# bernardomig/torch_semantic_segmentation

Measured on AMD Instinct MI355X. Metric: images/sec (train step) fastscnn 1024x2048 bs=8, higher is better.
Workload: dtype bf16; 1 GPU; fastscnn train step (zero_grad+fwd+CE(ignore 255)+bwd+AdamW), 8 x 3 x 1024 x 2048 per GPU, 19 classes, random-init weights; global_batch=8, parallelism=dp1, hip_graph=True, syncbn=False

## Files before the change

include/tss_hip.h:

```cpp
#ifndef TSS_HIP_H
#define TSS_HIP_H

#ifdef __cplusplus
extern "C" {
#endif

#define TSS_OK 0
#define TSS_ERR_DTYPE (-1)
#define TSS_ERR_SHAPE (-2)
#define TSS_ERR_ALIGN (-3)
#define TSS_ERR_HIP (-4)

#define TSS_F32 0
#define TSS_BF16 1

typedef struct tss_bn_bwd_job {
  const double* bstats; double count; const float* invstd; const float* gamma; int training; int accumulate;
  float* dgamma; float* dbeta; float* ga; float* gb; float* gce; int C;
  int xchg_world; int xchg_rank; void* xchg_peers[8]; void* xchg_counters;
} tss_bn_bwd_job;

enum {
  TSS_K_PWCONV_FWD = 0, TSS_K_PWCONV_BWD_DATA, TSS_K_PWCONV_BWD_WEIGHT,
  TSS_K_CONV3X3_FWD, TSS_K_CONV3X3_BWD_DATA, TSS_K_CONV3X3_BWD_WEIGHT,
  TSS_K_STEM_FWD, TSS_K_STEM_BWD_WEIGHT,
  TSS_K_DWCONV_FWD, TSS_K_DWCONV_BWD_DATA, TSS_K_DWCONV_BWD_WEIGHT,
  TSS_K_BN_FINALIZE, TSS_K_BN_BWD_FINALIZE, TSS_K_JOIN_FWD, TSS_K_JOIN_BWD,
  TSS_K_DROPOUT, TSS_K_BIAS_GRAD, TSS_K_ADAMW,
  TSS_K_BILINEAR_FWD, TSS_K_BILINEAR_BWD, TSS_K_BILINEAR_BWD_COLS, TSS_K_BILINEAR_PLANAR_FWD,
  TSS_K_UPSAMPLE_HEAD_FWD, TSS_K_UPSAMPLE_HEAD_BWD_ROWS, TSS_K_UPSAMPLE_HEAD_BWD_COLS,
  TSS_K_POOL_FWD, TSS_K_POOL_BWD, TSS_K_COPY,
  TSS_K_CE_FWD, TSS_K_CE_BWD, TSS_K_ARGMAX, TSS_K_UPSAMPLE_CE_FWD, TSS_K_UPSAMPLE_CE_BWD,
  TSS_K_RESIZE_FLIP_PLANAR, TSS_K_MULTISCALE_ARGMAX,
  TSS_K_SGD, TSS_K_GRAD_NORM,
  TSS_K_WIDE_CE_FWD, TSS_K_WIDE_CE_BWD, TSS_K_WIDE_ARGMAX, TSS_K_WIDE_MULTISCALE_ARGMAX,
  TSS_K_COUNT
};

int tss_version(void);
int tss_memset_zero(void* p, long bytes, void* stream);
const char* tss_last_error(void);
const char* tss_arch(void);
#define TSS_OPT_DISABLE_FAST_PATHS 1
int tss_set_option(int key, int value);
int tss_get_option(int key);

int tss_prof_enable(int on);
int tss_prof_reset(void);
int tss_prof_collect(void);
int tss_prof_get(int kernel_id, long* launches, double* total_ms, double* alg_bytes, double* flops);
long tss_prof_records(int* kernel_ids, double* ms, double* alg_bytes, long max_records);
const char* tss_prof_name(int kernel_id);
const char* tss_prof_symbol(int kernel_id);

int tss_pwconv_fwd(const void* x, long ldx, const float* in_mean, const float* in_scale, const float* in_bias, int in_relu,
                   const float* w, const void* w_bf16, const float* bias, void* y, long ldy, double* stats,
                   long P, int K, int N, int dtype, void* stream);
int tss_pwconv_fwd_joined(const void* x, long ldx, const float* in_mean, const float* in_scale, const float* in_bias, int in_relu,
// ... 210 lines not shown
int tss_bn_eval_affine(const float* gamma, const float* running_mean, const float* running_var,
                       float eps, float* mean_out, float* invstd_out, float* scale, int C, void* stream);
int tss_bn_eval_affine_batched(const long long* table, int njobs, int max_channels, void* stream);
int tss_bn_bwd_finalize(const double* bstats, double count, const float* invstd,
                        const float* gamma, int training, int accumulate, float* dgamma, float* dbeta,
                        float* ga, float* gb, float* gce, int C, void* stream);

int tss_slab_reduce(const double* slabs, double count, double* out, int C, void* stream);
int tss_bn_finalize_sync(const double* gsums, const float* gamma, float eps, float momentum, float* running_mean,
                         float* running_var, long long* num_batches_tracked, float* mean_out, float* invstd_out,
                         float* scale, int C, void* stream);
int tss_bn_bwd_finalize_sync(const double* bstats, const double* gsums, const float* invstd, const float* gamma,
                             int accumulate, float* dgamma, float* dbeta, float* ga, float* gb, float* gce, int C,
                             void* stream);

int tss_join_fwd(const void* a, long lda, const float* ma, const float* sa, const float* ba,
                 const void* b, long ldb, const float* mb, const float* sb, const float* bb,
                 void* out, long ldo, int relu, float drop_p, const unsigned long long* seed_slot,
                 long P, int C, int dtype, void* stream);
int tss_join_bwd(const void* dout, long lddo, const void* out, long ldo, int relu,
                 const void* a_raw, long lda, const float* mean_a, double* stats_a,
                 const void* b_raw, long ldb, const float* mean_b, double* stats_b,
                 void* e, long lde, float dout_scale, long P, int C, int dtype, void* stream);

int tss_dropout_tick(unsigned long long* counter, unsigned long long* seed_slot, void* stream);
int tss_dropout(const void* x, long ldx, void* y, long ldy, long P, int C, float p,
                const unsigned long long* seed_slot, int dtype, void* stream);
int tss_bias_grad(const void* e, long lde, long P, int N, float* dbias, int dtype, void* stream);
int tss_dropout_mask(const unsigned long long* counter, void* mask, long P, int C, float p, void* stream);
int tss_pwconv_drop_supported(long P, int K, int N, int dtype);
int tss_pwconv_fwd_drop(const void* x, long ldx, const float* in_mean, const float* in_scale, const float* in_bias, int in_relu,
                        const float* w, const void* w_bf16, const float* bias, void* y, long ldy,
                        const void* mask, float drop_p, unsigned long long* counter,
                        long P, int K, int N, int dtype, void* stream);
int tss_pwconv_bwd_fused_drop_supported(long P, int Cin, int Cout, int dtype);
int tss_pwconv_bwd_fused_drop_rows(long P);
int tss_pwconv_bwd_fused_drop(const void* e, long lde, const void* yraw, long ldyr, const float* ga, const float* gb, const float* gce,
                              const float* gmu, const float* w, const void* x, long ldx, const float* in_mean,
                              const float* in_scale, const float* in_bias, int in_relu, int x_pending, const void* mask, float drop_p,
                              void* e_in, long ldei, double* bstats, float* ws, float* bias_ws, long P, int Cin, int Cout, int dtype,
                              void* stream);
int tss_cast_weights(const long long* table, int njobs, int blocks_per_job, float* zero, long zero_n, void* stream);
int tss_adamw_step(float* params, const float* grads, float* exp_avg, float* exp_avg_sq, long n,
                   const float* lr, float beta1, float beta2, float eps, float weight_decay,
                   float* state, float grad_scale, float lr_host, long step_host, void* stream);

// ... 170 lines not shown
```

torch_semantic_segmentation_amd/_native.py:

```python
import ctypes
import os

import torch

_HERE = os.path.dirname(os.path.abspath(__file__))
LIB_PATH = os.environ.get('TSS_HIP_LIB') or os.path.join(_HERE, 'libtss_hip.so')

TSS_F32, TSS_BF16 = 0, 1
ERRORS = {-1: 'TSS_ERR_DTYPE (unsupported dtype)', -2: 'TSS_ERR_SHAPE (unsupported shape or pitch)',
          -3: 'TSS_ERR_ALIGN (pointer not 16-byte aligned)', -4: 'TSS_ERR_HIP (HIP launch error)'}

_P, _L, _I, _F, _D = ctypes.c_void_p, ctypes.c_long, ctypes.c_int, ctypes.c_float, ctypes.c_double

HEADER_PATH = os.path.join(os.path.dirname(_HERE), 'include', 'tss_hip.h')


def parse_header(path=HEADER_PATH):
    import re
    text = open(path).read()
    text = re.sub(r'/\*.*?\*/', ' ', text, flags=re.S)
    scalars = {'int': _I, 'long': _L, 'float': _F, 'double': _D}
    decls = {}
    for m in re.finditer(r'\b(int|long|const\s+char\s*\*)\s*(tss_\w+)\s*\(([^)]*)\)\s*;', text):
        ret, name, params = m.group(1), m.group(2), m.group(3).strip()
# ... 47 lines not shown
def stream():
    return torch.cuda.current_stream().cuda_stream


_slabs = None


def stat_slabs():
    global _slabs
    if _slabs is None:
        _slabs = lib().tss_stat_slabs()
    return _slabs


def dtype_code(dtype):
    if dtype == torch.float32:
        return TSS_F32
    if dtype == torch.bfloat16:
        return TSS_BF16
    raise TypeError('the HIP path computes in float32 or bfloat16 activations, got %s' % dtype)



K_COUNT = 41


def prof_enable(on=True):
    call('tss_prof_enable', 1 if on else 0)


def prof_reset():
    call('tss_prof_reset')


def prof_records(limit=100000):
    h = lib()
    ids = (ctypes.c_int * limit)()
    ms = (ctypes.c_double * limit)()
    by = (ctypes.c_double * limit)()
    n = min(h.tss_prof_records(ids, ms, by, limit), limit)
    return [(h.tss_prof_name(ids[i]).decode(), ms[i], by[i]) for i in range(n)]


def prof_table():
    call('tss_prof_collect')
    out = {}
    h = lib()
# ... 8 lines not shown
```

torch_semantic_segmentation_amd/csrc/bnfin.h:

```cpp
#pragma once
#include "common.h"

namespace tss_fin {

constexpr int FIN_CH = 8, FIN_RG = 4, FIN_WAVES = 4, FIN_NT = FIN_WAVES * 64;
static_assert(2 * FIN_CH * FIN_RG == 64, "one wave = row groups x 2 columns x channels");
__device__ __forceinline__ void slab_sum(const double* slabs, int C, int blk, double* s0, double* s1, int* c_out) {
  __shared__ double red[FIN_WAVES][64];
  const int lane = threadIdx.x & 63, wave = threadIdx.x >> 6;
  const int cl = lane & (FIN_CH - 1), hs = (lane / FIN_CH) & 1, rg = lane / (2 * FIN_CH);
  const int c = blk * FIN_CH + cl;
  const bool in = c < C;
  const double* col = slabs + (long)hs * C + (in ? c : 0);
  constexpr int RSTEP = FIN_WAVES * FIN_RG;
  constexpr int R = TSS_STAT_SLABS / RSTEP;
  static_assert(TSS_STAT_SLABS % RSTEP == 0, "slab rows must divide evenly");
  double acc = 0.0;
  double v[R];
#pragma unroll
  for (int u = 0; u < R; ++u) v[u] = col[(long)(wave * FIN_RG + rg + RSTEP * u) * 2 * C];
#pragma unroll
  for (int u = 0; u < R; ++u) acc += v[u];
  red[wave][lane] = in ? acc : 0.0;
  __syncthreads();
  double a = 0.0, b = 0.0;
  if (threadIdx.x < FIN_CH) {
#pragma unroll
    for (int w = 0; w < FIN_WAVES; ++w)
#pragma unroll
      for (int q = 0; q < FIN_RG; ++q) {
        a += red[w][q * 2 * FIN_CH + threadIdx.x];
        b += red[w][q * 2 * FIN_CH + FIN_CH + threadIdx.x];
      }
  }
  *s0 = a; *s1 = b; *c_out = blk * FIN_CH + threadIdx.x;
}


constexpr int XMAXB = 96;
constexpr int XCELL = 18;
constexpr int XSLOTS = 4;
constexpr int XMAXW = 8;
constexpr long XHEAD = 8;

__host__ __device__ inline long cell_off(int slot, int rank, int blk) { return XHEAD + (((long)slot * XMAXW + rank) * XMAXB + blk) * XCELL; }

struct Xchg {
  unsigned long long* peers[XMAXW];
  int rank, world;
  unsigned long long* ctr;
};

__device__ __forceinline__ void st_sys(unsigned long long* p, unsigned long long v) {
  __hip_atomic_store(p, v, __ATOMIC_RELAXED, __HIP_MEMORY_SCOPE_SYSTEM);
}
__device__ __forceinline__ unsigned long long ld_sys(const unsigned long long* p) {
  return __hip_atomic_load(p, __ATOMIC_RELAXED, __HIP_MEMORY_SCOPE_SYSTEM);
}
// ... 84 lines not shown
```

torch_semantic_segmentation_amd/csrc/pointwise.hip:

```cpp
#include <cstdlib>
#include "common.h"
#include "bnfin.h"

namespace {

constexpr int NT = 256;

using namespace tss_fin;

__global__ __launch_bounds__(FIN_NT) void bn_finalize_kernel(const double* sums, double count, const float* gamma,
                                   float eps, float momentum, float* running_mean, float* running_var,
                                   long long* num_batches, float* mean_out, float* invstd_out,
                                   float* scale, int C) {
  if (blockIdx.x == 0 && threadIdx.x == 0 && num_batches) *num_batches += 1;
  const int cp = min(blockIdx.x * FIN_CH + (int)(threadIdx.x & (FIN_CH - 1)), C - 1);
  const float g_in = (gamma ? gamma : mean_out)[cp];
  const float rm_in = (running_mean ? running_mean : mean_out)[cp];
  const float rv_in = (running_var ? running_var : mean_out)[cp];
  double ssum, ssq;
  int c;
  slab_sum(sums, C, blockIdx.x, &ssum, &ssq, &c);
  if (threadIdx.x >= FIN_CH || c >= C) return;
  const double mean = ssum / count;
  double var = ssq / count - mean * mean;
  if (var < 0.0) var = 0.0;
  const float invstd = (float)(1.0 / sqrt(var + (double)eps));
  const float g = gamma ? g_in : 1.f;
  const float m = (float)mean;
  mean_out[c] = m;
  invstd_out[c] = invstd;
  scale[c] = g * invstd;
  if (running_mean) running_mean[c] = (1.f - momentum) * rm_in + momentum * m;
  if (running_var) {
    const double unbiased = count > 1.0 ? var * count / (count - 1.0) : var;
    running_var[c] = (1.f - momentum) * rv_in + momentum * (float)unbiased;
  }
}

__global__ __launch_bounds__(FIN_NT) void slab_reduce_kernel(const double* slabs, double count, double* out, int C) {
  double s0, s1;
  int c;
  slab_sum(slabs, C, blockIdx.x, &s0, &s1, &c);
  if (blockIdx.x == 0 && threadIdx.x == 0) out[2 * C] = count;
  if (threadIdx.x >= FIN_CH || c >= C) return;
  out[c] = s0;
  out[C + c] = s1;
}

__global__ void bn_finalize_sync_kernel(const double* gsums, const float* gamma, float eps, float momentum,
                                        float* running_mean, float* running_var, long long* num_batches,
                                        float* mean_out, float* invstd_out, float* scale, int C) {
  const int c = blockIdx.x * blockDim.x + threadIdx.x;
  if (c == 0 && num_batches) *num_batches += 1;
  if (c >= C) return;
  const double count = gsums[2 * C];
  const double mean = gsums[c] / count;
  double var = gsums[C + c] / count - mean * mean;
  if (var < 0.0) var = 0.0;
  const float invstd = (float)(1.0 / sqrt(var + (double)eps));
// ... 74 lines not shown
  V4<float>::load(q + 4, v + 4);
#pragma unroll
  for (int j = 0; j < 8; ++j) out[j] = (has && active) ? v[j] : dflt;
}

__device__ __forceinline__ void philox4x32(uint32_t c0, uint32_t c1, uint32_t k0, uint32_t k1, uint32_t out[4]) {
  uint32_t c[4] = {c0, c1, 0u, 0u};
#pragma unroll
  for (int r = 0; r < 10; ++r) {
    const uint64_t p0 = (uint64_t)0xD2511F53u * c[0];
    const uint64_t p1 = (uint64_t)0xCD9E8D57u * c[2];
    const uint32_t n0 = (uint32_t)(p1 >> 32) ^ c[1] ^ k0;
    const uint32_t n1 = (uint32_t)p1;
    const uint32_t n2 = (uint32_t)(p0 >> 32) ^ c[3] ^ k1;
    const uint32_t n3 = (uint32_t)p0;
    c[0] = n0; c[1] = n1; c[2] = n2; c[3] = n3;
    k0 += 0x9E3779B9u; k1 += 0xBB67AE85u;
  }
  out[0] = c[0]; out[1] = c[1]; out[2] = c[2]; out[3] = c[3];
}

__global__ void dropout_tick_kernel(unsigned long long* counter, unsigned long long* slot) {
  if (threadIdx.x == 0 && blockIdx.x == 0) { *slot = *counter; *counter += 1ull; }
}

template <typename T>
__global__ __launch_bounds__(NT) void join_fwd_kernel(const JoinArgs g) {
  const int tid = threadIdx.x;
  const int cg = tid % g.CV, pl = tid / g.CV;
  if (pl >= g.NPL) return;
  const int c0 = cg * 8;
  const T* a = reinterpret_cast<const T*>(g.a);
  const T* b = reinterpret_cast<const T*>(g.b);
  T* out = reinterpret_cast<T*>(g.out);
  float ma[8], sa[8], ba[8], mb[8], sb[8], bb[8];
  const float* safe = reinterpret_cast<const float*>(g.a);
  coef8(g.sa, safe, c0, true, 1.f, sa);
  coef8(g.sa ? g.ma : nullptr, safe, c0, true, 0.f, ma);
  coef8(g.sa ? g.ba : nullptr, safe, c0, true, 0.f, ba);
  coef8(g.sb, safe, c0, true, 1.f, sb);
  coef8(g.sb ? g.mb : nullptr, safe, c0, true, 0.f, mb);
  coef8(g.sb ? g.bb : nullptr, safe, c0, true, 0.f, bb);
  const long stride = (long)gridDim.x * g.NPL;
  const float relu_lo = g.relu ? 0.f : -__builtin_inff();
  const unsigned long long dseed = g.seed_slot ? *g.seed_slot : 0ull;
  const uint32_t dk0 = (uint32_t)dseed, dk1 = (uint32_t)(dseed >> 32) ^ 0x5EEDu;
// ... 21 lines not shown
      V8<T>::unpack(rb[u], uu);
#pragma unroll
      for (int j = 0; j < 8; ++j) {
        v[j] = (v[j] - ma[j]) * sa[j] + ba[j];
        if (hb) v[j] += (uu[j] - mb[j]) * sb[j] + bb[j];
        v[j] = fmaxf(v[j], relu_lo);
      }
      if (g.seed_slot) {
        uint32_t r0[4], r1[4];
        const uint64_t ctr = (uint64_t)(p * g.C + c0) >> 2;
        philox4x32((uint32_t)ctr, (uint32_t)(ctr >> 32), dk0, dk1, r0);
        philox4x32((uint32_t)(ctr + 1), (uint32_t)((ctr + 1) >> 32), dk0, dk1, r1);
#pragma unroll
        for (int j = 0; j < 4; ++j) {
          v[j] = (r0[j] >= dthresh) ? V8<T>::round(v[j]) * dinv : 0.f;
          v[4 + j] = (r1[j] >= dthresh) ? V8<T>::round(v[4 + j]) * dinv : 0.f;
        }
      }
      V8<T>::store(out + p * g.ldo + c0, v);
    }
  }
}

template <typename T> struct StatAcc { typedef float type; };
template <> struct StatAcc<float> { typedef double type; };

template <typename T>
__global__ __launch_bounds__(NT) void join_bwd_kernel(const JoinArgs g) {
  typedef typename StatAcc<T>::type A;
  __shared__ __align__(16) unsigned char smem[NT * 8 * 3 * sizeof(double)];
  const int tid = threadIdx.x;
  const int cg = tid % g.CV, pl = tid / g.CV;
  const bool active = pl < g.NPL;
  const int c0 = cg * 8;
  const T* dout = reinterpret_cast<const T*>(g.dout);
  const T* out = reinterpret_cast<const T*>(g.out);
  const T* a = reinterpret_cast<const T*>(g.a);
  const T* b = reinterpret_cast<const T*>(g.b);
  T* e = reinterpret_cast<T*>(g.e);
  A s0[8], sA[8], sB[8];
  float ma[8], mb[8];
#pragma unroll
  for (int j = 0; j < 8; ++j) { s0[j] = 0; sA[j] = 0; sB[j] = 0; }
  const float* safe = reinterpret_cast<const float*>(g.dout);
  coef8(g.ma, safe, c0, active, 0.f, ma);
  coef8(g.mb, safe, c0, active, 0.f, mb);
// ... 283 lines not shown
  return tss::check_last("bn_bwd_finalize");
}

int tss_join_fwd(const void* a, long lda, const float* ma, const float* sa, const float* ba,
                 const void* b, long ldb, const float* mb, const float* sb, const float* bb,
                 void* out, long ldo, int relu, float drop_p, const unsigned long long* seed_slot,
                 long P, int C, int dtype, void* stream) {
  TSS_CHECK_DTYPE(dtype);
  TSS_REQUIRE((lda % 8) == 0 && lda >= C && (ldo % 8) == 0 && ldo >= C && (!b || ((ldb % 8) == 0 && ldb >= C)), TSS_ERR_SHAPE);
  TSS_REQUIRE(!seed_slot || (relu && drop_p > 0.f && drop_p < 1.f), TSS_ERR_SHAPE);
  TSS_REQUIRE(tss::aligned16(a) && tss::aligned16(out) && tss::aligned16(b), TSS_ERR_ALIGN);
  JoinArgs g = {};
  g.a = a; g.lda = lda; g.ma = ma; g.sa = sa; g.ba = ba; g.b = b; g.ldb = ldb; g.mb = mb; g.sb = sb; g.bb = bb;
  g.out = out; g.ldo = ldo; g.relu = relu; g.P = P; g.C = C;
  g.drop_p = seed_slot ? drop_p : 0.f; g.seed_slot = seed_slot; g.dscale = 1.f;
  int threads, grid;
  static const long fwd_blocks = getenv("TSS_JOIN_FWD_BLOCKS") ? atol(getenv("TSS_JOIN_FWD_BLOCKS")) : 512;
  const int rc = join_geometry(g, &threads, &grid, fwd_blocks);
  if (rc) return rc;
  if (P == 0) return TSS_OK;
  tss::ProfScope prof(TSS_K_JOIN_FWD, (hipStream_t)stream, (double)P * C * (b ? 3 : 2) * tss::esz(dtype), 0);
  TSS_WITH_DTYPE(dtype, hipLaunchKernelGGL(join_fwd_kernel<TT>, dim3(grid), dim3(threads), 0, (hipStream_t)stream, g));
  return tss::check_last("join_fwd");
}

int tss_join_bwd(const void* dout, long lddo, const void* out, long ldo, int relu,
                 const void* a_raw, long lda, const float* mean_a, double* stats_a,
                 const void* b_raw, long ldb, const float* mean_b, double* stats_b,
                 void* e, long lde, float dout_scale, long P, int C, int dtype, void* stream) {
  TSS_CHECK_DTYPE(dtype);
  TSS_REQUIRE((lddo % 8) == 0 && lddo >= C && (!relu || (out && (ldo % 8) == 0 && ldo >= C)), TSS_ERR_SHAPE);
  TSS_REQUIRE(dout_scale > 0.f && (dout_scale == 1.f || relu), TSS_ERR_SHAPE);
  TSS_REQUIRE((!stats_a || (a_raw && (lda % 8) == 0 && lda >= C)) && (!stats_b || (b_raw && (ldb % 8) == 0 && ldb >= C)), TSS_ERR_SHAPE);
  TSS_REQUIRE(!e || ((lde % 8) == 0 && lde >= C), TSS_ERR_SHAPE);
  TSS_REQUIRE(tss::aligned16(dout) && tss::aligned16(e), TSS_ERR_ALIGN);
  JoinArgs g = {};
  g.dout = dout; g.lddo = lddo; g.out = const_cast<void*>(out); g.ldo = ldo; g.relu = relu;
  g.a = a_raw; g.lda = lda; g.ma = mean_a; g.stats_a = stats_a; g.b = b_raw; g.ldb = ldb; g.mb = mean_b; g.stats_b = stats_b;
  g.e = e; g.lde = lde; g.P = P; g.C = C; g.dscale = dout_scale;
  int threads, grid;
  const int rc = join_geometry(g, &threads, &grid);
  if (rc) return rc;
  if (P == 0) return TSS_OK;
  const int nt = 1 + (relu ? 1 : 0) + (e ? 1 : 0) + (stats_a ? 1 : 0) + (stats_b ? 1 : 0);
  tss::ProfScope prof(TSS_K_JOIN_BWD, (hipStream_t)stream, (double)P * C * nt * tss::esz(dtype), 0);
  TSS_WITH_DTYPE(dtype, hipLaunchKernelGGL(join_bwd_kernel<TT>, dim3(grid), dim3(threads), 0, (hipStream_t)stream, g));
// ... 88 lines not shown
```

torch_semantic_segmentation_amd/csrc/prof.cpp:

```cpp
#include <mutex>
#include <vector>

#include "common.h"

namespace {

struct KernelInfo { const char* name; const char* symbol; };
const KernelInfo kInfo[TSS_K_COUNT] = {
    {"pwconv_fwd", "pwfast_kernel<false>|pwfast_mc_kernel<false>|convgemm_kernel"},
    {"pwconv_bwd_data", "pwfast_kernel<true>|pwfast_mc_kernel<true>|pwbwd_kernel|pwsweep_kernel|convgemm_kernel"},
    {"pwconv_bwd_weight", "wgfast_kernel|wgrad_kernel"},
    {"conv3x3_fwd", "conv3x3_wstat_kernel|conv3x3_stream_kernel|conv3x3_lean_kernel<false>|fc1d_kernel|convgemm_kernel<fwd>"}, {"conv3x3_bwd_data", "conv3x3_lean_kernel<true>|fc1d_kernel|convgemm_kernel<bwd>"}, {"conv3x3_bwd_weight", "fc1d_wgrad_kernel|wgrad_kernel"},
    {"stem3x3_fwd", "stem_fwd_mfma_kernel|convgemm_kernel"}, {"stem3x3_bwd_weight", "stem_wgrad_mfma_kernel|stem_wgrad_kernel"},
    {"dwconv3x3_fwd", "dw_fwd_roll_kernel|dw_fwd_strip_kernel"}, {"dwconv3x3_bwd_data", "dw_bwd_roll_s1_kernel|dw_bwd_roll_s2_kernel|dw_bwd_data_strip_kernel"},
    {"dwconv3x3_bwd_weight", "dw_bwd_weight_strip_kernel"},
    {"bn_finalize", "bn_finalize_kernel"}, {"bn_bwd_finalize", "bn_bwd_finalize_kernel"},
    {"join_fwd", "join_fwd_kernel"}, {"join_bwd", "join_bwd_kernel"},
    {"dropout", "dropout_kernel"}, {"bias_grad", "colsum_kernel"}, {"adamw", "adamw_kernel"},
    {"bilinear_nhwc_fwd", "bilinear_nhwc_fwd_kernel|ppm_concat_fwd_kernel"}, {"bilinear_nhwc_bwd_rows", "bilinear_nhwc_bwd_rows_kernel|ppm_concat_bwd_kernel"},
    {"bilinear_nhwc_bwd_cols", "bilinear_nhwc_bwd_cols_kernel"},
    {"bilinear_planar_fwd", "bilinear_planar_fwd_kernel"},
    {"upsample_head_fwd", "upsample_head_fwd_kernel"}, {"upsample_head_bwd_rows", "upsample_head_bwd_rows_kernel"},
    {"upsample_head_bwd_cols", "upsample_head_bwd_cols_kernel"},
    {"adaptive_pool_fwd", "adaptive_pool_fwd_kernel|ppm_pool_fwd_kernel"}, {"adaptive_pool_bwd", "adaptive_pool_bwd_kernel|ppm_pool_bwd_kernel"},
    {"copy_nhwc", "copy_nhwc_kernel"},
    {"cross_entropy_fwd", "ce_fwd_kernel"}, {"cross_entropy_bwd", "ce_bwd_kernel"}, {"argmax_confusion", "argmax_confusion_kernel"},
    {"upsample_ce_fwd", "upsample_ce_onepass_kernel"}, {"upsample_ce_bwd", "upsample_ce_gather_kernel"},
    {"resize_flip_planar", "resize_flip_planar_kernel"}, {"multiscale_argmax_confusion", "multiscale_argmax_kernel"},
    {"sgd", "sgd_kernel"}, {"grad_norm", "grad_sqnorm_kernel|grad_sqnorm_final_kernel"},
    {"upsample_ce_wide_fwd", "wide_ce_kernel"}, {"upsample_ce_wide_bwd", "wide_ce_gather_kernel"},
    {"argmax_confusion_wide", "wide_upsample_argmax_kernel|wide_planar_argmax_kernel"},
    {"multiscale_argmax_confusion_wide", "wide_multiscale_argmax_kernel"},
};

struct Rec { int kid; hipEvent_t a, b; double bytes, flops; };
struct Total { long launches; double ms, bytes, flops; };
struct Done { int kid; double ms, bytes; };
std::vector<Done> g_done;

std::mutex g_mu;
bool g_enabled = false;
std::vector<Rec> g_recs;
std::vector<hipEvent_t> g_pool;
Total g_tot[TSS_K_COUNT];
thread_local char g_err[256] = "";

hipEvent_t get_event() {
  if (!g_pool.empty()) { hipEvent_t e = g_pool.back(); g_pool.pop_back(); return e; }
  hipEvent_t e;
  (void)hipEventCreate(&e);
  return e;
}

}

// ... 97 lines not shown
```

torch_semantic_segmentation_amd/models/lednet.py:

```python
from collections import OrderedDict

import torch
from torch import nn
from torch.nn import functional as F

from .. import ops
from ._fused import FusedSequential, HipModel, run

__all__ = ['LedNet', 'lednet', 'APNModule', 'DownsamplingBlock', 'SSnbtBlock', 'FactorizedConvBlock', 'ConvBlock', 'channel_shuffle']


def lednet(in_channels, out_channels):
    return LedNet(in_channels, out_channels)


class LedNet(HipModel):

    def __init__(self, in_channels, out_channels):
        super().__init__()
        self.encoder = FusedSequential(OrderedDict([
            ('layer1', FusedSequential(
                DownsamplingBlock(in_channels, 32),
                SSnbtBlock(32, 32, dropout_p=0.03),
                SSnbtBlock(32, 32, dropout_p=0.03),
# ... 44 lines not shown
                sh.running_mean[:C].copy_(bn.running_mean)
                sh.running_var[:C].copy_(bn.running_var)
                sh.num_batches_tracked.copy_(bn.num_batches_tracked)
        return sh

    def leave(self, bn):
        if bn.training and bn.track_running_stats and bn.running_mean is not None:
            C, sh = bn.num_features, self.shim
            with torch.no_grad():
                bn.running_mean.copy_(sh.running_mean[:C])
                bn.running_var.copy_(sh.running_var[:C])
                bn.num_batches_tracked.copy_(sh.num_batches_tracked)


def _padded_block(x, block, cp, pad):
    conv, bn = block[0], block[1]
    C = conv.out_channels
    if C == cp:
        return run(block, x)
    w = F.pad(conv.weight, (0, 0, 0, 0, 0, 0, 0, cp - C))
    gamma, beta = F.pad(bn.weight, (0, cp - C), value=1.0), F.pad(bn.bias, (0, cp - C))
    sh = pad.enter(bn, cp)
    out = ops.conv_unit(x, conv, sh, True, weight=w, gamma=gamma, beta=beta, cout=cp)
    pad.leave(bn)
    return out


class APNModule(nn.Module):

    def __init__(self, in_channels, out_channels):
        super().__init__()
        self.conv1 = ConvBlock(in_channels, in_channels, 3, 1, stride=2)
        self.conv2 = ConvBlock(in_channels, in_channels, 5, 2, stride=2)
        self.conv3 = ConvBlock(in_channels, in_channels, 7, 3, stride=2)
        self.level1 = ConvBlock(in_channels, out_channels, 1)
        self.level2 = ConvBlock(in_channels, out_channels, 1)
        self.level3 = ConvBlock(in_channels, out_channels, 1)
        self.level4 = ConvBlock(in_channels, out_channels, 1)
        self.level5 = ConvBlock(in_channels, out_channels, 1)
        self.__dict__['_pads'] = [_PadBN() for _ in range(5)]

    def forward(self, input):
        x = ops.to_nhwc(ops.materialize(input))
        C = self.level1[0].out_channels
        cp = ops.round_up(C, 8)
        pads = self.__dict__['_pads']
# ... 94 lines not shown
```

torch_semantic_segmentation_amd/ops.py:

```python
import collections
import ctypes
import math
import os
import threading

import torch
from torch.autograd import Function
from torch.nn.modules.batchnorm import _BatchNorm

from . import _native as N

call, ptr, stream = N.call, N.ptr, N.stream



_DIRECT = [False]


class direct_grads:

    def __init__(self, enabled=True):
        self.enabled = bool(enabled)

    def __enter__(self):
        self.prev = _DIRECT[0]
        _DIRECT[0] = self.enabled
        return self

    def __exit__(self, *exc):
        _DIRECT[0] = self.prev
        return False


overlap_wgrad = os.environ.get('TSS_OVERLAP_WGRAD', '0') == '1'
fuse_dw_backward = os.environ.get('TSS_FUSE_DW_BWD', '0') == '1'
overlap_max_elems = int(os.environ.get('TSS_OVERLAP_MAX', str(48 << 20)))
overlap_min_elems = int(os.environ.get('TSS_OVERLAP_MIN', '0'))
batch_dw_reductions = os.environ.get('TSS_BATCH_DW_REDUCE', '1') == '1'
fuse_pw_backward = os.environ.get('TSS_PW_BWD_FUSED', '1') != '0'
sweep_pw_backward = os.environ.get('TSS_PW_SWEEP', '1') != '0'
postpone_wgrad = os.environ.get('TSS_POSTPONE_WGRAD', '1') != '0'
unfold_1d_wgrad = os.environ.get('TSS_FC1D_WGRAD', '1') != '0'
_CONST_ROWS = {}


def _per_device(cache, dev, make, stale=lambda got: False):
    key = (dev.type, dev.index)
    if key not in cache or stale(cache[key]):
        cache[key] = make()
    return cache[key]


def _const_rows(dev, n):
    m = max(768, n)
    return _per_device(_CONST_ROWS, dev, lambda: (torch.ones(m, dtype=torch.float32, device=dev), torch.zeros(m, dtype=torch.float32, device=dev)),
                       stale=lambda got: got[0].numel() < n)
_overlap_depth = [0]
postpone_in_overlap = os.environ.get('TSS_POSTPONE_OVERLAPPED', '0') == '1'


class _Pass:
    __slots__ = ('dw', 'wg', 'red')

    def __init__(self):
        self.dw = []
        self.wg = {}
        self.red = {}


_passes = {}
_lock = threading.RLock()


class BnBwdJob(ctypes.Structure):
    _fields_ = [('bstats', ctypes.c_void_p), ('count', ctypes.c_double), ('invstd', ctypes.c_void_p), ('gamma', ctypes.c_void_p),
                ('training', ctypes.c_int), ('accumulate', ctypes.c_int), ('dgamma', ctypes.c_void_p), ('dbeta', ctypes.c_void_p),
                ('ga', ctypes.c_void_p), ('gb', ctypes.c_void_p), ('gce', ctypes.c_void_p), ('C', ctypes.c_int),
                ('xchg_world', ctypes.c_int), ('xchg_rank', ctypes.c_int), ('xchg_peers', ctypes.c_void_p * 8), ('xchg_counters', ctypes.c_void_p)]


def _backward_task():
    try:
        task = torch._C._current_graph_task_id()
    except AttributeError:
        return -1
    if task == -1:
        return -1
    with _lock:
        if task not in _passes:
            try:
                torch.autograd.variable.Variable._execution_engine.queue_callback(lambda _t=task: _end_of_backward(_t))
            except Exception:
                return -1
            for old in sorted(_passes)[:-15]:
                del _passes[old]
            _passes[task] = _Pass()
    return task


def _cur_pass():
    task = _backward_task()
# ... 442 lines not shown


def _check_device(t):
    if not t.is_cuda:
        raise RuntimeError('torch_semantic_segmentation_amd runs on the MI355X HIP path only: got a %s tensor. '
                           'There is no CPU fallback (the CPU oracle lives in oracle/, for tests).' % t.device)
    if t.device.index is not None and t.device.index != torch.cuda.current_device():
        raise RuntimeError('tensor lives on cuda:%d but the current device is cuda:%d; wrap the call in '
                           'torch.cuda.device(%d) (one process per GPU is the supported layout)'
                           % (t.device.index, torch.cuda.current_device(), t.device.index))
    N.lib()


def ld(t):
    return t.stride(3)


def npix(t):
    return t.shape[0] * t.shape[2] * t.shape[3]



class BNLink:
    __slots__ = ('C', 'count', 'training', 'gamma', 'beta', 'vec', 'scale', 'mean', 'invstd',
                 'ga', 'gb', 'gce', 'stats', 'bstats', 'consumed', 'sync')

    def __init__(self, C, count, training, gamma, beta, device, slabs=True):
        self.C, self.count, self.training, self.gamma, self.beta = C, count, training, gamma, beta
        self.vec = torch.empty((6, C), dtype=torch.float32, device=device)
        self.mean, self.invstd, self.scale, self.ga, self.gb, self.gce = self.vec.unbind(0)
        if slabs:
            both = torch.empty((2, N.stat_slabs(), 2 * C), dtype=torch.float64, device=device)
            self.stats, self.bstats = both[0], both[1]
        else:
            self.stats = self.bstats = None
        self.consumed = False
        self.sync = None


class Deferred:
    __slots__ = ('raw', 'link', 'relu')

    def __init__(self, raw, link=None, relu=False):
        self.raw, self.link, self.relu = raw, link, relu

    @property
    def shape(self):
        return self.raw.shape


    def take(self):
        if self.link is not None:
            if self.link.consumed:
                raise RuntimeError('a deferred BatchNorm output may feed exactly one consumer; materialize it first')
            self.link.consumed = True
        return self


class SyncBatchNorm(torch.nn.BatchNorm2d):
    process_group = None
# ... 385 lines not shown

def _bias_grad_into(e, P, Cout, out, dt, st):
    if Cout <= 64:
        call('tss_bias_grad', ptr(e), ld(e), P, Cout, ptr(out), dt, st)
    else:
        out.add_(_colsum(e, Cout, st))


def _finalize_forward(link, bn, training, P, Cout, gamma, st):
    if training:
        track = bn.track_running_stats and bn.running_mean is not None
        rbuf = _F32Buffers(bn, track)
        run_args = (ptr(rbuf.mean), ptr(rbuf.var),
                    ptr(bn.num_batches_tracked) if (track and bn.num_batches_tracked is not None) else None)
        link.sync = _sync_group(bn)
        ex = _exchange(link.sync, link.stats.device) if (link.sync is not None and Cout <= 768) else None
        if ex is not None:
            call('tss_bn_finalize_xchg', ptr(link.stats), float(P), ex.peers, ex.rank, ex.world, ptr(ex.counters), ptr(gamma),
                 float(bn.eps), float(bn.momentum), *run_args, ptr(link.mean), ptr(link.invstd), ptr(link.scale), Cout, st)
        elif link.sync is not None:
            gs = _allreduce_stats(link.stats, P, Cout, link.sync, st)
            call('tss_bn_finalize_sync', ptr(gs), ptr(gamma), float(bn.eps), float(bn.momentum), *run_args,
                 ptr(link.mean), ptr(link.invstd), ptr(link.scale), Cout, st)
        else:
            call('tss_bn_finalize', ptr(link.stats), float(P), ptr(gamma), float(bn.eps),
                 float(bn.momentum), *run_args, ptr(link.mean), ptr(link.invstd), ptr(link.scale), Cout, st)
        rbuf.close()
    else:
        pre = _EVAL_AFFINES.get(id(bn)) if _EVAL_AFFINES else None
        if pre is not None:
            link.mean, link.invstd, link.scale = pre.unbind(0)
        else:
            rbuf = _F32Buffers(bn, True)
            call('tss_bn_eval_affine', ptr(gamma), ptr(rbuf.mean), ptr(rbuf.var),
                 float(bn.eps), ptr(link.mean), ptr(link.invstd), ptr(link.scale), Cout, st)


def _frozen_link(bn, C, P, dev, st):
    gamma, beta = _f32(bn.weight), _f32(bn.bias)
    link = BNLink(C, P, False, gamma, beta, dev, slabs=False)
    _finalize_forward(link, bn, False, P, C, gamma, st)
    return link, beta


_FwdArgs = collections.namedtuple('_FwdArgs', 'cfg x weight bias y aff stats B Hin Win Cout P s d dt dev st')

# ... 520 lines not shown
            raise RuntimeError('join: operand b carries a pending ReLU; materialize it first')
        if b.raw.shape != a.raw.shape or b.raw.dtype != a.raw.dtype:
            raise RuntimeError('join: operands differ in shape/dtype: %s vs %s' % (a.raw.shape, b.raw.shape))
        braw, cfg.b_link = b.raw, b.link
    cfg.res_fork = fork if b is not None else None
    cfg.j_a = cfg.fused_e = None
    out = JoinFn.apply(a.raw, braw, cfg)
    if (fuse_join_backward and cfg.relu and not cfg.drop_p and cfg.a_link is not None and cfg.b_link is None and out.requires_grad
            and out.dtype == torch.bfloat16 and not N.fast_paths_disabled()):
        cfg.j_a = a.raw
        _hand(out, _JOIN, cfg)
    return out


class JoinFn(Function):
    @staticmethod
    def forward(ctx, a, b, cfg):
        out = new_nhwc(*a.shape, a.dtype, a.device)
        al, bl = cfg.a_link, cfg.b_link
        slot = None
        if cfg.drop_p:
            slot = torch.empty(1, dtype=torch.int64, device=a.device)
            call('tss_dropout_tick', ptr(_dropout_counter(a.device)), ptr(slot), stream())
        call('tss_join_fwd', ptr(a), ld(a), *_aff(al), ptr(b), ld(b) if b is not None else 0, *_aff(bl),
             ptr(out), ld(out), int(cfg.relu), cfg.drop_p, ptr(slot), npix(a), a.shape[1], N.dtype_code(a.dtype), stream())
        ctx.cfg = cfg
        ctx.has_b = b is not None
        ctx.save_for_backward(a if al is not None else None, b if bl is not None else None,
                              out if cfg.relu else None)
        return out

    @staticmethod
    def backward(ctx, dout):
        cfg = ctx.cfg
        a, b, out = ctx.saved_tensors
        fe = cfg.fused_e
        cfg.fused_e = None
        if (fe is not None and dout.data_ptr() == fe.data_ptr() and dout.shape == fe.shape and dout.dtype == fe.dtype
                and dout.stride() == fe.stride()):
            fork = cfg.res_fork
            if fork is not None and ctx.has_b:
                fork.g2 = dout
            return dout, (dout if ctx.has_b else None), None
        del fe
        dout = to_nhwc(dout)
        al, bl = cfg.a_link, cfg.b_link
        e = new_nhwc(*dout.shape, dout.dtype, dout.device) if cfg.relu else None
        if cfg.relu or al is not None or bl is not None:
# ... 1819 lines not shown
```

Before: 1734 images/sec.

## Fuse BatchNorm finalize into join forward kernel for small activations

BatchNorm statistics finalization is deferred: the forward pass records a pending finalize job instead of launching a separate kernel. When the next join (residual add/ReLU/dropout) consumes that BN output and the tensor is small (≤3 MiB), a new fused kernel reduces the stat slabs per channel group, writes mean/invstd/scale and running stats, and applies the affine join in the same launch. Any other consumer triggers the finalize lazily through property accessors. This removes a kernel launch and a dependency per BN in the small low-resolution layers. The cost is redundant slab reduction in every block and extra complexity in lazy state handling.

```diff
diff --git a/include/tss_hip.h b/include/tss_hip.h
--- a/include/tss_hip.h
+++ b/include/tss_hip.h
@@ -19,6 +19,12 @@
   float* dgamma; float* dbeta; float* ga; float* gb; float* gce; int C;
   int xchg_world; int xchg_rank; void* xchg_peers[8]; void* xchg_counters;
 } tss_bn_bwd_job;
+
+typedef struct tss_bn_fin_job {
+  const double* sums; double count; const float* gamma; float eps; float momentum;
+  float* running_mean; float* running_var; long long* num_batches_tracked;
+  float* mean_out; float* invstd_out; float* scale;
+} tss_bn_fin_job;
 
 enum {
   TSS_K_PWCONV_FWD = 0, TSS_K_PWCONV_BWD_DATA, TSS_K_PWCONV_BWD_WEIGHT,
@@ -34,6 +40,7 @@
   TSS_K_RESIZE_FLIP_PLANAR, TSS_K_MULTISCALE_ARGMAX,
   TSS_K_SGD, TSS_K_GRAD_NORM,
   TSS_K_WIDE_CE_FWD, TSS_K_WIDE_CE_BWD, TSS_K_WIDE_ARGMAX, TSS_K_WIDE_MULTISCALE_ARGMAX,
+  TSS_K_JOIN_FWD_FIN,
   TSS_K_COUNT
 };
 
@@ -290,6 +297,11 @@
                  const void* a_raw, long lda, const float* mean_a, double* stats_a,
                  const void* b_raw, long ldb, const float* mean_b, double* stats_b,
                  void* e, long lde, float dout_scale, long P, int C, int dtype, void* stream);
+int tss_join_fwd_fin(const void* a, long lda, const tss_bn_fin_job* fin_a, const float* ma, const float* sa, const float* ba,
+                     const void* b, long ldb, const tss_bn_fin_job* fin_b, const float* mb, const float* sb, const float* bb,
+                     void* out, long ldo, int relu, float drop_p, const unsigned long long* seed_slot,
+                     long P, int C, int dtype, void* stream);
+int tss_join_fwd_fin_preferred(long P, int C, int has_b, int dtype);
 
 int tss_dropout_tick(unsigned long long* counter, unsigned long long* seed_slot, void* stream);
 int tss_dropout(const void* x, long ldx, void* y, long ldy, long P, int C, float p,
diff --git a/torch_semantic_segmentation_amd/_native.py b/torch_semantic_segmentation_amd/_native.py
--- a/torch_semantic_segmentation_amd/_native.py
+++ b/torch_semantic_segmentation_amd/_native.py
@@ -93,7 +93,7 @@
 
 
 
-K_COUNT = 41
+K_COUNT = 42
 
 
 def prof_enable(on=True):
diff --git a/torch_semantic_segmentation_amd/csrc/bnfin.h b/torch_semantic_segmentation_amd/csrc/bnfin.h
--- a/torch_semantic_segmentation_amd/csrc/bnfin.h
+++ b/torch_semantic_segmentation_amd/csrc/bnfin.h
@@ -34,6 +34,30 @@
       }
   }
   *s0 = a; *s1 = b; *c_out = blk * FIN_CH + threadIdx.x;
+}
+
+__device__ __forceinline__ void bn_finalize_tail(double ssum, double ssq, double count, const float* gamma, float g_in, float eps,
+                                                 float momentum, float* running_mean, float rm_in, float* running_var, float rv_in,
+                                                 float* mean_out, float* invstd_out, float* scale_out, int c, bool write,
+                                                 float* m_ret, float* scale_ret) {
+  const double mean = ssum / count;
+  double var = ssq / count - mean * mean;
+  if (var < 0.0) var = 0.0;
+  const float invstd = (float)(1.0 / sqrt(var + (double)eps));
+  const float g = gamma ? g_in : 1.f;
+  const float m = (float)mean;
+  if (write) {
+    mean_out[c] = m;
+    invstd_out[c] = invstd;
+    scale_out[c] = g * invstd;
+    if (running_mean) running_mean[c] = (1.f - momentum) * rm_in + momentum * m;
+    if (running_var) {
+      const double unbiased = count > 1.0 ? var * count / (count - 1.0) : var;
+      running_var[c] = (1.f - momentum) * rv_in + momentum * (float)unbiased;
+    }
+  }
+  *m_ret = m;
+  *scale_ret = g * invstd;
 }
 
 
diff --git a/torch_semantic_segmentation_amd/csrc/pointwise.hip b/torch_semantic_segmentation_amd/csrc/pointwise.hip
--- a/torch_semantic_segmentation_amd/csrc/pointwise.hip
+++ b/torch_semantic_segmentation_amd/csrc/pointwise.hip
@@ -21,20 +21,9 @@
   int c;
   slab_sum(sums, C, blockIdx.x, &ssum, &ssq, &c);
   if (threadIdx.x >= FIN_CH || c >= C) return;
-  const double mean = ssum / count;
-  double var = ssq / count - mean * mean;
-  if (var < 0.0) var = 0.0;
-  const float invstd = (float)(1.0 / sqrt(var + (double)eps));
-  const float g = gamma ? g_in : 1.f;
-  const float m = (float)mean;
-  mean_out[c] = m;
-  invstd_out[c] = invstd;
-  scale[c] = g * invstd;
-  if (running_mean) running_mean[c] = (1.f - momentum) * rm_in + momentum * m;
-  if (running_var) {
-    const double unbiased = count > 1.0 ? var * count / (count - 1.0) : var;
-    running_var[c] = (1.f - momentum) * rv_in + momentum * (float)unbiased;
-  }
+  float m, sc;
+  bn_finalize_tail(ssum, ssq, count, gamma, g_in, eps, momentum, running_mean, rm_in, running_var, rv_in, mean_out, invstd_out, scale,
+                   c, true, &m, &sc);
 }
 
 __global__ __launch_bounds__(FIN_NT) void slab_reduce_kernel(const double* slabs, double count, double* out, int C) {
@@ -155,6 +144,46 @@
 
 __global__ void dropout_tick_kernel(unsigned long long* counter, unsigned long long* slot) {
   if (threadIdx.x == 0 && blockIdx.x == 0) { *slot = *counter; *counter += 1ull; }
+}
+
+struct JoinCoef {
+  float ma[8], sa[8], ba[8], mb[8], sb[8], bb[8];
+  float relu_lo, dinv;
+  uint32_t dk0, dk1, dthresh;
+};
+
+__device__ __forceinline__ void join_scalars(const JoinArgs& g, JoinCoef& k) {
+  k.relu_lo = g.relu ? 0.f : -__builtin_inff();
+  const unsigned long long dseed = g.seed_slot ? *g.seed_slot : 0ull;
+  k.dk0 = (uint32_t)dseed; k.dk1 = (uint32_t)(dseed >> 32) ^ 0x5EEDu;
+  k.dinv = 1.f / (1.f - g.drop_p);
+  k.dthresh = (uint32_t)((double)g.drop_p * 4294967296.0);
+}
+
+template <typename T>
+__device__ __forceinline__ void join_pixel(const JoinArgs& g, const typename V8<T>::Raw& ra, const typename V8<T>::Raw& rb,
+                                           const JoinCoef& k, bool hb, long p, int c0, T* out) {
+  float v[8], uu[8];
+  V8<T>::unpack(ra, v);
+  V8<T>::unpack(rb, uu);
+#pragma unroll
+  for (int j = 0; j < 8; ++j) {
+    v[j] = (v[j] - k.ma[j]) * k.sa[j] + k.ba[j];
+    if (hb) v[j] += (uu[j] - k.mb[j]) * k.sb[j] + k.bb[j];
+    v[j] = fmaxf(v[j], k.relu_lo);
+  }
+  if (g.seed_slot) {
+    uint32_t r0[4], r1[4];
+    const uint64_t ctr = (uint64_t)(p * g.C + c0) >> 2;
+    philox4x32((uint32_t)ctr, (uint32_t)(ctr >> 32), k.dk0, k.dk1, r0);
+    philox4x32((uint32_t)(ctr + 1), (uint32_t)((ctr + 1) >> 32), k.dk0, k.dk1, r1);
+#pragma unroll
+    for (int j = 0; j < 4; ++j) {
+      v[j] = (r0[j] >= k.dthresh) ? V8<T>::round(v[j]) * k.dinv : 0.f;
+      v[4 + j] = (r1[j] >= k.dthresh) ? V8<T>::round(v[4 + j]) * k.dinv : 0.f;
+    }
+  }
+  V8<T>::store(out + p * g.ldo + c0, v);
 }
 
 template <typename T>
@@ -222,6 +251,105 @@
   }
 }
 
+struct FinLink {
+  const double* slabs; double count; const float* gamma; float eps, momentum;
+  float* running_mean; float* running_var; long long* num_batches; float* mean; float* invstd; float* scale;
+};
+struct JoinFinArgs { JoinArgs g; FinLink fa, fb; int G; };
+
+__device__ __forceinline__ void join_fin_link(const FinLink& f, int C, int grp, bool writer, float* m_lds, float* s_lds) {
+  const int cp = min(grp * FIN_CH + (int)(threadIdx.x & (FIN_CH - 1)), C - 1);
+  const float* dummy = reinterpret_cast<const float*>(f.slabs);
+  const float g_in = (f.gamma ? f.gamma : dummy)[cp];
+  float rm_in = 0.f, rv_in = 0.f;
+  if (writer) {
+    rm_in = (f.running_mean ? f.running_mean : dummy)[cp];
+    rv_in = (f.running_var ? f.running_var : dummy)[cp];
+  }
+  double ssum, ssq;
+  int c;
+  slab_sum(f.slabs, C, grp, &ssum, &ssq, &c);
+  if (threadIdx.x < FIN_CH) {
+    float m = 0.f, sc = 0.f;
+    if (c < C)
+      bn_finalize_tail(ssum, ssq, f.count, f.gamma, g_in, f.eps, f.momentum, f.running_mean, rm_in, f.running_var, rv_in, f.mean,
+                       f.invstd, f.scale, c, writer, &m, &sc);
+    m_lds[threadIdx.x] = m;
+    s_lds[threadIdx.x] = sc;
+  }
+}
+
+template <typename T>
+__global__ __launch_bounds__(NT) void join_fwd_fin_kernel(const JoinFinArgs f) {
+  __shared__ float cf[4][FIN_CH];
+  const JoinArgs& g = f.g;
+  const int xcd = blockIdx.x & 7, kb = blockIdx.x >> 3;
+  const int grp = kb % f.G, slice = (kb / f.G) * 8 + xcd;
+  const long stride = (long)(gridDim.x / f.G) * NT;
+  long p0 = (long)slice * NT + threadIdx.x;
+  if ((long)slice * NT >= g.P) return;
+  const bool writer = slice == 0;
+  const int c0 = grp * 8;
+  const T* a = reinterpret_cast<const T*>(g.a);
+  const T* b = reinterpret_cast<const T*>(g.b);
+  T* out = reinterpret_cast<T*>(g.out);
+  const bool hb = b != nullptr;
+  const T* b2 = hb ? b : a;
+  const long ldb2 = hb ? g.ldb : g.lda;
+  constexpr int JU = 4;
+  typename V8<T>::Raw ra[JU], rb[JU];
+#pragma unroll
+  for (int u = 0; u < JU; ++u) {
+    const long p = p0 + u * stride;
+    const long q = p < g.P ? p : g.P - 1;
+    ra[u] = V8<T>::load_raw(a + q * g.lda + c0);
+    rb[u] = V8<T>::load_raw(b2 + q * ldb2 + c0);
+  }
+  if (blockIdx.x == 0 && threadIdx.x == 0) {
+    if (f.fa.slabs && f.fa.num_batches) *f.fa.num_batches += 1;
+    if (f.fb.slabs && f.fb.num_batches) *f.fb.num_batches += 1;
+  }
+  JoinCoef k8;
+  const float* safe = reinterpret_cast<const float*>(g.a);
+  coef8(f.fa.slabs ? nullptr : g.sa, safe, c0, true, 1.f, k8.sa);
+  coef8((f.fa.slabs || !g.sa) ? nullptr : g.ma, safe, c0, true, 0.f, k8.ma);
+  coef8((f.fa.slabs || g.sa) ? g.ba : nullptr, safe, c0, true, 0.f, k8.ba);
+  coef8(f.fb.slabs ? nullptr : g.sb, safe, c0, true, 1.f, k8.sb);
+  coef8((f.fb.slabs || !g.sb) ? nullptr : g.mb, safe, c0, true, 0.f, k8.mb);
+  coef8((f.fb.slabs || g.sb) ? g.bb : nullptr, safe, c0, true, 0.f, k8.bb);
+  if (f.fa.slabs) join_fin_link(f.fa, g.C, grp, writer, cf[0], cf[1]);
+  if (f.fa.slabs && f.fb.slabs) __syncthreads();
+  if (f.fb.slabs) join_fin_link(f.fb, g.C, grp, writer, cf[2], cf[3]);
+  __syncthreads();
+  if (f.fa.slabs) {
+#pragma unroll
+    for (int j = 0; j < 8; ++j) { k8.ma[j] = cf[0][j]; k8.sa[j] = cf[1][j]; }
+  }
+  if (f.fb.slabs) {
+#pragma unroll
+    for (int j = 0; j < 8; ++j) { k8.mb[j] = cf[2][j]; k8.sb[j] = cf[3][j]; }
+  }
+  join_scalars(g, k8);
+  while (p0 < g.P) {
+#pragma unroll
+    for (int u = 0; u < JU; ++u) {
+      const long p = p0 + u * stride;
+      if (p >= g.P) break;
+      join_pixel<T>(g, ra[u], rb[u], k8, hb, p, c0, out);
+    }
+    p0 += stride * JU;
+    if (p0 < g.P) {
+#pragma unroll
+      for (int u = 0; u < JU; ++u) {
+        const long p = p0 + u * stride;
+        const long q = p < g.P ? p : p0;
+        ra[u] = V8<T>::load_raw(a + q * g.lda + c0);
+        rb[u] = V8<T>::load_raw(b2 + q * ldb2 + c0);
+      }
+    }
+  }
+}
+
 template <typename T> struct StatAcc { typedef float type; };
 template <> struct StatAcc<float> { typedef double type; };
 
@@ -551,6 +679,60 @@
   tss::ProfScope prof(TSS_K_JOIN_FWD, (hipStream_t)stream, (double)P * C * (b ? 3 : 2) * tss::esz(dtype), 0);
   TSS_WITH_DTYPE(dtype, hipLaunchKernelGGL(join_fwd_kernel<TT>, dim3(grid), dim3(threads), 0, (hipStream_t)stream, g));
   return tss::check_last("join_fwd");
+}
+
+constexpr long FINJOIN_MAX_BYTES = 3l << 20;
+
+int tss_join_fwd_fin_preferred(long P, int C, int has_b, int dtype) {
+  (void)has_b;
+  if ((dtype != TSS_F32 && dtype != TSS_BF16) || P <= 0 || C <= 0 || (C % 8) != 0 || C > NT * 8) return 0;
+  static const long max_bytes = getenv("TSS_FINJOIN_MAX_BYTES") ? atol(getenv("TSS_FINJOIN_MAX_BYTES")) : FINJOIN_MAX_BYTES;
+  return P * C * (long)tss::esz(dtype) <= max_bytes ? 1 : 0;
+}
+
+int tss_join_fwd_fin(const void* a, long lda, const tss_bn_fin_job* fin_a, const float* ma, const float* sa, const float* ba,
+                     const void* b, long ldb, const tss_bn_fin_job* fin_b, const float* mb, const float* sb, const float* bb,
+                     void* out, long ldo, int relu, float drop_p, const unsigned long long* seed_slot,
+                     long P, int C, int dtype, void* stream) {
+  TSS_CHECK_DTYPE(dtype);
+  TSS_REQUIRE(C > 0 && (C % 8) == 0 && C <= NT * 8 && P >= 0, TSS_ERR_SHAPE);
+  TSS_REQUIRE((lda % 8) == 0 && lda >= C && (ldo % 8) == 0 && ldo >= C && (!b || ((ldb % 8) == 0 && ldb >= C)), TSS_ERR_SHAPE);
+  TSS_REQUIRE(!seed_slot || (relu && drop_p > 0.f && drop_p < 1.f), TSS_ERR_SHAPE);
+  TSS_REQUIRE((fin_a || fin_b) && (!fin_b || b), TSS_ERR_SHAPE);
+  TSS_REQUIRE(tss::aligned16(a) && tss::aligned16(out) && tss::aligned16(b), TSS_ERR_ALIGN);
+  JoinFinArgs f = {};
+  JoinArgs& g = f.g;
+  g.a = a; g.lda = lda; g.ma = ma; g.sa = sa; g.ba = ba; g.b = b; g.ldb = ldb; g.mb = mb; g.sb = sb; g.bb = bb;
+  g.out = out; g.ldo = ldo; g.relu = relu; g.P = P; g.C = C;
+  g.drop_p = seed_slot ? drop_p : 0.f; g.seed_slot = seed_slot; g.dscale = 1.f;
+  const tss_bn_fin_job* jobs[2] = {fin_a, fin_b};
+  FinLink* links[2] = {&f.fa, &f.fb};
+  for (int i = 0; i < 2; ++i) {
+    const tss_bn_fin_job* j = jobs[i];
+    if (!j) continue;
+    TSS_REQUIRE(j->sums && j->count >= 1.0 && j->mean_out && j->invstd_out && j->scale, TSS_ERR_SHAPE);
+    *links[i] = FinLink{j->sums, j->count, j->gamma, j->eps, j->momentum, j->running_mean, j->running_var, j->num_batches_tracked,
+                        j->mean_out, j->invstd_out, j->scale};
+  }
+  if (P == 0) {
+    for (int i = 0; i < 2; ++i) {
+      const tss_bn_fin_job* j = jobs[i];
+      if (!j) continue;
+      const int rc = tss_bn_finalize(j->sums, j->count, j->gamma, j->eps, j->momentum, j->running_mean, j->running_var,
+                                     j->num_batches_tracked, j->mean_out, j->invstd_out, j->scale, C, stream);
+      if (rc) return rc;
+    }
+    return TSS_OK;
+  }
+  static const long blocks = getenv("TSS_JOIN_FIN_BLOCKS") ? atol(getenv("TSS_JOIN_FIN_BLOCKS")) : 256;
+  f.G = C / 8;
+  long S = (P + NT * 4 - 1) / (NT * 4);
+  const long cap = blocks / f.G > 8 ? blocks / f.G : 8;
+  if (S > cap) S = cap;
+  S = (S + 7) / 8 * 8;
+  tss::ProfScope prof(TSS_K_JOIN_FWD_FIN, (hipStream_t)stream, (double)P * C * (b ? 3 : 2) * tss::esz(dtype) + 40.0 * C * ((fin_a ? 1 : 0) + (fin_b ? 1 : 0)), 0);
+  TSS_WITH_DTYPE(dtype, hipLaunchKernelGGL(join_fwd_fin_kernel<TT>, dim3((int)(S * f.G)), dim3(NT), 0, (hipStream_t)stream, f));
+  return tss::check_last("join_fwd_fin");
 }
 
 int tss_join_bwd(const void* dout, long lddo, const void* out, long ldo, int relu,
diff --git a/torch_semantic_segmentation_amd/csrc/prof.cpp b/torch_semantic_segmentation_amd/csrc/prof.cpp
--- a/torch_semantic_segmentation_amd/csrc/prof.cpp
+++ b/torch_semantic_segmentation_amd/csrc/prof.cpp
@@ -31,6 +31,7 @@
     {"upsample_ce_wide_fwd", "wide_ce_kernel"}, {"upsample_ce_wide_bwd", "wide_ce_gather_kernel"},
     {"argmax_confusion_wide", "wide_upsample_argmax_kernel|wide_planar_argmax_kernel"},
     {"multiscale_argmax_confusion_wide", "wide_multiscale_argmax_kernel"},
+    {"join_fwd_fin", "join_fwd_fin_kernel"},
 };
 
 struct Rec { int kid; hipEvent_t a, b; double bytes, flops; };
diff --git a/torch_semantic_segmentation_amd/models/lednet.py b/torch_semantic_segmentation_amd/models/lednet.py
--- a/torch_semantic_segmentation_amd/models/lednet.py
+++ b/torch_semantic_segmentation_amd/models/lednet.py
@@ -90,6 +90,8 @@
     gamma, beta = F.pad(bn.weight, (0, cp - C), value=1.0), F.pad(bn.bias, (0, cp - C))
     sh = pad.enter(bn, cp)
     out = ops.conv_unit(x, conv, sh, True, weight=w, gamma=gamma, beta=beta, cout=cp)
+    if out.link is not None:
+        out.link.finalize_now()
     pad.leave(bn)
     return out
 
diff --git a/torch_semantic_segmentation_amd/ops.py b/torch_semantic_segmentation_amd/ops.py
--- a/torch_semantic_segmentation_amd/ops.py
+++ b/torch_semantic_segmentation_amd/ops.py
@@ -40,6 +40,7 @@
 fuse_pw_backward = os.environ.get('TSS_PW_BWD_FUSED', '1') != '0'
 sweep_pw_backward = os.environ.get('TSS_PW_SWEEP', '1') != '0'
 postpone_wgrad = os.environ.get('TSS_POSTPONE_WGRAD', '1') != '0'
+fuse_fin_join = os.environ.get('TSS_FUSE_FIN_JOIN', '1') != '0'
 unfold_1d_wgrad = os.environ.get('TSS_FC1D_WGRAD', '1') != '0'
 _CONST_ROWS = {}
 
@@ -77,6 +78,13 @@
                 ('training', ctypes.c_int), ('accumulate', ctypes.c_int), ('dgamma', ctypes.c_void_p), ('dbeta', ctypes.c_void_p),
                 ('ga', ctypes.c_void_p), ('gb', ctypes.c_void_p), ('gce', ctypes.c_void_p), ('C', ctypes.c_int),
                 ('xchg_world', ctypes.c_int), ('xchg_rank', ctypes.c_int), ('xchg_peers', ctypes.c_void_p * 8), ('xchg_counters', ctypes.c_void_p)]
+
+
+class BnFinJob(ctypes.Structure):
+    _fields_ = [('sums', ctypes.c_void_p), ('count', ctypes.c_double), ('gamma', ctypes.c_void_p), ('eps', ctypes.c_float),
+                ('momentum', ctypes.c_float), ('running_mean', ctypes.c_void_p), ('running_var', ctypes.c_void_p),
+                ('num_batches_tracked', ctypes.c_void_p), ('mean_out', ctypes.c_void_p), ('invstd_out', ctypes.c_void_p),
+                ('scale', ctypes.c_void_p)]
 
 
 def _backward_task():
@@ -565,13 +573,14 @@
 
 
 class BNLink:
-    __slots__ = ('C', 'count', 'training', 'gamma', 'beta', 'vec', 'scale', 'mean', 'invstd',
-                 'ga', 'gb', 'gce', 'stats', 'bstats', 'consumed', 'sync')
+    __slots__ = ('C', 'count', 'training', 'gamma', 'beta', 'vec', '_scale', '_mean', '_invstd',
+                 'ga', 'gb', 'gce', 'stats', 'bstats', 'consumed', 'sync', 'pending')
 
     def __init__(self, C, count, training, gamma, beta, device, slabs=True):
         self.C, self.count, self.training, self.gamma, self.beta = C, count, training, gamma, beta
         self.vec = torch.empty((6, C), dtype=torch.float32, device=device)
-        self.mean, self.invstd, self.scale, self.ga, self.gb, self.gce = self.vec.unbind(0)
+        self.pending = None
+        self._mean, self._invstd, self._scale, self.ga, self.gb, self.gce = self.vec.unbind(0)
         if slabs:
             both = torch.empty((2, N.stat_slabs(), 2 * C), dtype=torch.float64, device=device)
             self.stats, self.bstats = both[0], both[1]
@@ -579,6 +588,29 @@
             self.stats = self.bstats = None
         self.consumed = False
         self.sync = None
+
+    def finalize_now(self):
+        job = self.pending
+        if job is not None:
+            self.pending = None
+            call('tss_bn_finalize', job.sums, job.count, job.gamma, job.eps, job.momentum, job.running_mean, job.running_var,
+                 job.num_batches_tracked, job.mean_out, job.invstd_out, job.scale, self.C, stream())
+
+    def take_pending(self):
+        job, self.pending = self.pending, None
+        return job
+
+    def _coef(name):
+        def get(self):
+            self.finalize_now()
+            return getattr(self, name)
+
+        def put(self, value):
+            setattr(self, name, value)
+        return property(get, put)
+
+    mean, invstd, scale = _coef('_mean'), _coef('_invstd'), _coef('_scale')
+    del _coef
 
 
 class Deferred:
@@ -1010,6 +1042,11 @@
             gs = _allreduce_stats(link.stats, P, Cout, link.sync, st)
             call('tss_bn_finalize_sync', ptr(gs), ptr(gamma), float(bn.eps), float(bn.momentum), *run_args,
                  ptr(link.mean), ptr(link.invstd), ptr(link.scale), Cout, st)
+        elif fuse_fin_join and not rbuf.pairs and link.stats is not None:
+            job = BnFinJob(ptr(link.stats), float(P), ptr(gamma), float(bn.eps), float(bn.momentum), *run_args,
+                           ptr(link._mean), ptr(link._invstd), ptr(link._scale))
+            job.keep = (gamma, bn.running_mean, bn.running_var, bn.num_batches_tracked)
+            link.pending = job
         else:
             call('tss_bn_finalize', ptr(link.stats), float(P), ptr(gamma), float(bn.eps),
                  float(bn.momentum), *run_args, ptr(link.mean), ptr(link.invstd), ptr(link.scale), Cout, st)
@@ -1576,8 +1613,17 @@
         if cfg.drop_p:
             slot = torch.empty(1, dtype=torch.int64, device=a.device)
             call('tss_dropout_tick', ptr(_dropout_counter(a.device)), ptr(slot), stream())
-        call('tss_join_fwd', ptr(a), ld(a), *_aff(al), ptr(b), ld(b) if b is not None else 0, *_aff(bl),
-             ptr(out), ld(out), int(cfg.relu), cfg.drop_p, ptr(slot), npix(a), a.shape[1], N.dtype_code(a.dtype), stream())
+        P, C, dt = npix(a), a.shape[1], N.dtype_code(a.dtype)
+        fused = (fuse_fin_join and any(l is not None and l.pending is not None for l in (al, bl)) and not N.fast_paths_disabled()
+                 and N.lib().tss_join_fwd_fin_preferred(P, C, int(b is not None), dt))
+        if fused:
+            fa, fb = (l.take_pending() if l is not None else None for l in (al, bl))
+            call('tss_join_fwd_fin', ptr(a), ld(a), ctypes.byref(fa) if fa is not None else None, *_aff(al),
+                 ptr(b), ld(b) if b is not None else 0, ctypes.byref(fb) if fb is not None else None, *_aff(bl),
+                 ptr(out), ld(out), int(cfg.relu), cfg.drop_p, ptr(slot), P, C, dt, stream())
+        else:
+            call('tss_join_fwd', ptr(a), ld(a), *_aff(al), ptr(b), ld(b) if b is not None else 0, *_aff(bl),
+                 ptr(out), ld(out), int(cfg.relu), cfg.drop_p, ptr(slot), P, C, dt, stream())
         ctx.cfg = cfg
         ctx.has_b = b is not None
         ctx.save_for_backward(a if al is not None else None, b if bl is not None else None,
```

Result: no change. 1730 images/sec (-0.3%).
